# Lcressot/fhe-string-bounty

Hardware: AMD Instinct MI355X
Metric: PBS/sec (whole node) (higher is better)
Workload: dtype f64

## Files before the change

### fhe-string-bounty_amd/csrc/engine.h

```cpp
#pragma once
#include <hip/hip_runtime.h>
#include <stdint.h>

#include <map>
#include <mutex>
#include <string>
#include <vector>

#include "../../include/fhestr.h"

#define FHESTR_KERNEL_REVISION "r04.2"

namespace fhe {

inline uint32_t n_ggsw(const fhe_params_t& p) {
    return p.grouping_factor > 1 ? p.n / p.grouping_factor * (1u << p.grouping_factor) : p.n;
}
inline uint64_t multi_bit_key_bit(const uint64_t* group_bits, uint32_t g, uint32_t sel) {
    uint64_t prod = 1;
    for (uint32_t b = 0; b < g; b++) prod *= group_bits[b] ^ (((sel >> (g - 1 - b)) & 1) ^ 1);
    return prod;
}

void aes128_round_keys(const uint8_t key[16], uint8_t rk[11][16]);
const uint8_t* aes_sbox();

extern thread_local std::string g_last_error;
int fail(const std::string& msg);

struct BrVariant;

uint64_t fill_accumulator(const fhe_params_t& p, const uint64_t* table, std::vector<uint64_t>& acc);
void fill_accumulator_torus(const fhe_params_t& p, const uint64_t* box_values, std::vector<uint64_t>& acc);

struct EngineEnv {
    int log2_points = 0;
    int wide_fair = -1;
    int keep_busy = -1;
    int overlap_streams = -1;
    int ks_mfma = -1;
    int ks_chunks = -1;
    int cluster_mode = -2;
    int cluster_spin_limit = -1;
    int multibit_combine_max = -1;
    int cluster_test_fault = -1;
    int dense_per_cu = -1;
    int cluster_fallback = -1;
    static EngineEnv read();
};

struct Engine {
    std::recursive_mutex mu;
    fhe_params_t p{};
    int device = 0;
    hipStream_t stream = nullptr;
    hipStream_t own_stream = nullptr;
    std::map<std::vector<uint64_t>, uint32_t> lut_dedup;
    hipEvent_t ev[3] = {nullptr, nullptr, nullptr};
    std::vector<hipEvent_t> ring;
    size_t ring_used = 0;
    const BrVariant* variant = nullptr;
    const BrVariant* variant_large = nullptr;
    int cu_count = 256;
    int pipeline = 0;
    hipStream_t ks_stream = nullptr;
    hipEvent_t pipe_ev[5] = {nullptr, nullptr, nullptr, nullptr, nullptr};
    hipEvent_t pipe_input_ready = nullptr;
    const void* pipe_out[2] = {nullptr, nullptr};
    size_t pipe_out_bytes[2] = {0, 0};
    static constexpr int OVL_MAX = 4;
    int ovl_streams = 2;
    uint32_t wide_fair_shift = 13;
    uint32_t dense_per_cu = 2;
    bool keep_busy = false;
    hipStream_t ovl_stream[OVL_MAX] = {nullptr, nullptr, nullptr, nullptr};
    hipEvent_t ovl_done[OVL_MAX] = {nullptr, nullptr, nullptr, nullptr};
    struct ByteRange { const char* lo; const char* hi; };
    std::vector<ByteRange> ovl_ins[OVL_MAX], ovl_outs[OVL_MAX];
    uint64_t* ovl_small[OVL_MAX] = {nullptr, nullptr, nullptr, nullptr};
    size_t ovl_cap_small[OVL_MAX] = {0, 0, 0, 0};
    int8_t* ovl_digits[OVL_MAX] = {nullptr, nullptr, nullptr, nullptr};
    size_t ovl_cap_digits[OVL_MAX] = {0, 0, 0, 0};
    int sync_all_streams();
    void end_pipeline_run();
    uint64_t pipe_calls = 0;
    int shadow_fit = -1;
    uint32_t multibit_combine_max = 64;

    uint32_t* d_ksk_packed = nullptr;
    uint64_t* d_ksk_rowsum = nullptr;
    int8_t* d_ksk_mfma = nullptr;
    int8_t* d_ks_digits = nullptr;
    size_t cap_ks_digits = 0;
    bool ks_mfma_enabled = true;
    double* d_fbsk = nullptr;
    double* d_fbsk_dense = nullptr;
    uint64_t* d_luts = nullptr;
    size_t luts_cap = 0;
    uint32_t n_luts = 0;

    uint64_t *d_in = nullptr, *d_small = nullptr, *d_small2 = nullptr, *d_out = nullptr, *d_pool = nullptr;
    uint32_t* d_idx = nullptr;
    uint32_t* d_slot_exp = nullptr;
    size_t multibit_workspace_cap = 0;
    void* d_meta = nullptr;
    void* d_ws = nullptr;
    size_t cap_ws = 0;
    void* d_cluster_ws = nullptr;
    size_t cap_cluster_ws = 0;
    void* d_cluster_ctl = nullptr;
    bool cluster_unchecked = false;
    uint32_t cluster_last = 0;
    bool cluster_fallback = true;
    uint32_t cluster_fallbacks = 0;
    uint32_t cluster_last_error = 0;
    int cluster_mode = -1;
    uint32_t cluster_max_batch = 0xFFFFFFFFu;
    uint32_t ks_chunks_override = 0;
    int xcd_per_cu = -1;
    uint32_t xcd_auto_max = 16;
    uint32_t cluster_spin_limit = 1u << 22;
    uint32_t cluster_test_fault = 0;
    int cluster_check();
    size_t cap_in = 0, cap_small = 0, cap_small2 = 0, cap_out = 0, cap_idx = 0, cap_pool = 0, cap_meta = 0;

    static int create(const fhe_params_t& p, int device, Engine** out);
    ~Engine();
    int use();
    int set_variant(int logR);
    int load_keys(const uint64_t* bsk_std, const uint64_t* ksk);
    int load_seeded_keys(const uint8_t ksk_seed[16], const uint64_t* ksk_bodies, const uint8_t bsk_seed[16], const uint64_t* bsk_bodies,
                         uint64_t* bsk_std_out, uint64_t* ksk_out);
    int expand_seeded_lwe(const uint8_t* seeds, const uint64_t* bodies, uint32_t count, uint64_t* d_out, uint64_t* host_out);
    int generate_keys(const uint64_t* glwe_sk, const uint64_t* small_sk, const uint8_t seed[32],
                      uint64_t* bsk_std_out, uint64_t* ksk_out);
    int install_keys(uint64_t* d_ksk_std, uint64_t* d_bsk_std);
    int convert_polys(const uint64_t* d_std, double* d_out, uint32_t n_polys);
    int cluster_settle(const uint64_t* d_sm, const uint32_t* d_lut_idx, uint64_t* d_big, uint32_t count);
    int probe_slot_exponents();
    uint64_t fill_accumulator(const uint64_t* table, std::vector<uint64_t>& acc) const { return fhe::fill_accumulator(p, table, acc); }
    int lut_upload_dedup(const std::vector<uint64_t>& acc, uint32_t* id);
    int set_stream(hipStream_t s, bool use_own);
    int lut_upload(const uint64_t* acc, uint32_t* id);
    int lut_download(uint32_t id, uint64_t* acc);
    int ensure_batch(uint32_t count);
    int check_lut_idx(const uint32_t* lut_idx, uint32_t count) const;

    int launch_keyswitch(const uint64_t* d_big, uint64_t* d_sm, uint32_t count, hipStream_t on = nullptr, bool shadow = false, int digits_slot = 0);
    int launch_blind_rotate(const uint64_t* d_sm, const uint32_t* d_lut_idx, uint64_t* d_big, uint32_t count, hipStream_t on = nullptr, bool two_per_cu = false);
    bool shadow_keyswitch_fits();
    int ks_pbs_dev(const uint64_t* d_big_in, const uint32_t* d_lut_idx, uint64_t* d_big_out, uint32_t count, bool allow_pipeline = false);
    int ks_pbs_host(const uint64_t* in, const uint32_t* lut_idx, uint64_t* out, uint32_t count);
    int keyswitch_host(const uint64_t* in, uint64_t* out_small, uint32_t count);
    int pbs_host(const uint64_t* in_small, const uint32_t* lut_idx, uint64_t* out, uint32_t count);
    int pbs_ks_host(const uint64_t* in_small, const uint32_t* lut_idx, uint64_t* out_small, uint32_t count);
    int lincomb_dev(const uint64_t* d_pool, const uint32_t* d_off, const uint32_t* d_src,
                    const int32_t* d_coeff, const uint64_t* d_cst, uint64_t* d_out, uint32_t jobs);
    int lincomb_batch_dev(const uint64_t* d_pool, const uint32_t* d_off, const uint32_t* d_src, const int32_t* d_coeff,
                          const uint64_t* d_cst, uint64_t* d_out, uint32_t jobs, uint32_t instances, uint32_t src_slot, uint32_t src_inst,
                          uint32_t out_job, uint32_t out_inst, const uint32_t* d_lut_in, uint32_t* d_lut_out);
    int restride_dev(const uint64_t* d_in, uint64_t* d_out, uint32_t slots, uint32_t instances, uint32_t in_slot, uint32_t in_inst,
                     uint32_t out_slot, uint32_t out_inst);
    int lincomb_host(const uint64_t* pool, uint32_t pool_count, const uint32_t* off, const uint32_t* src,
                     const int32_t* coeff, const uint64_t* cst, uint64_t* out, uint32_t jobs);
    int last_kernel_ms(float ms[2]);
    int kernel_times(double total_ms[2], uint32_t* calls, bool reset);
    int synchronize();
};

int params_supported(const fhe_params_t& p);

}

struct fhe_plan;
struct fhe_engine {
    fhe::Engine* impl;
    std::vector<std::pair<std::string, fhe_plan*>> str_plans;
};
```

### fhe-string-bounty_amd/csrc/pbs_kernels.hip.h

```cpp
#pragma once
#include <type_traits>
#include "negacyclic_fft.hip.h"

namespace fhe {

#ifdef FHESTR_WALL
__device__ unsigned long long g_wall[4096 * 2];
#endif
#ifdef FHESTR_STAMPS
constexpr int STAMP_SEGS = 10;
__device__ unsigned long long g_stamps[4096 * 8 * STAMP_SEGS];
#define FHE_STAMP_DECL unsigned long long stamp_acc[STAMP_SEGS] = {}; unsigned long long stamp_prev = 0
#define FHE_STAMP(idx)                                                                                   \
    do {                                                                                                 \
        __builtin_amdgcn_sched_barrier(0);                                                               \
        unsigned long long _t;                                                                           \
        asm volatile("s_memtime %0\n\ts_waitcnt lgkmcnt(0)" : "=s"(_t)::"memory");                       \
        __builtin_amdgcn_sched_barrier(0);                                                               \
        if ((idx) >= 0) stamp_acc[(idx) < 0 ? 0 : (idx)] += _t - stamp_prev;                             \
        stamp_prev = _t;                                                                                 \
    } while (0)
#else
#define FHE_STAMP_DECL do {} while (0)
#define FHE_STAMP(idx) do {} while (0)
#endif

__device__ uint32_t g_cu_tickets[2048];

struct BlindRotateArgs {
    const uint64_t* lwe_small;
    const uint32_t* lut_idx;
    const uint64_t* luts;
    const double* fbsk;
    uint64_t* lwe_out;
    uint32_t n;
    uint32_t base_log;
    uint32_t batch;
    uint32_t grouping;
    uint32_t fair_shift;
};

__device__ __forceinline__ uint32_t decomp_init_state(uint64_t x, uint32_t bL) {
    uint32_t t = (uint32_t)(x >> (63 - bL));
    return ((t + 1u) >> 1) & ((1u << bL) - 1u);
}
__device__ __forceinline__ int32_t decomp_next_digit(uint32_t& state, uint32_t base_log) {
    const uint32_t mask = (1u << base_log) - 1u;
    uint32_t res = state & mask;
    state >>= base_log;
    uint32_t carry = ((res - 1u) | state) & res;
    carry >>= base_log - 1;
    state += carry;
    return (int32_t)(res - (carry << base_log));
}
__device__ __forceinline__ uint64_t decomp_init_state64(uint64_t x, uint32_t bL) {
    const uint64_t t = x >> (63 - bL);
    return ((t + 1ull) >> 1) & ((1ull << bL) - 1ull);
}
__device__ __forceinline__ int32_t decomp_next_digit64(uint64_t& state, uint32_t base_log) {
    const uint64_t mask = (1ull << base_log) - 1ull;
    uint64_t res = state & mask;
    state >>= base_log;
    uint64_t carry = ((res - 1ull) | state) & res;
    carry >>= base_log - 1;
    state += carry;
    return (int32_t)(uint32_t)(res - (carry << base_log));
}
__device__ __forceinline__ int32_t decomp_single_digit(uint64_t x, uint32_t b) {
    const uint32_t t = (uint32_t)(x >> 32) >> (31 - b);
    const uint32_t res = __builtin_amdgcn_ubfe(t + 1u, 1u, b);
    const uint32_t half = 1u << (b - 1);
    return (int32_t)(res - ((res + (half - 1u)) & (half << 1)));
}
__device__ __forceinline__ uint32_t decomp_bias_constant(uint32_t b) {
    uint32_t c = 0x80000000u - (1u << (31 - b));
    asm volatile("" : "+s"(c));
    return c;
}
__device__ __forceinline__ uint32_t decomp_single_biased(uint64_t x, uint32_t b, uint32_t bias_constant) {
    const uint32_t hi = (uint32_t)(x >> 32);
    return __builtin_amdgcn_ubfe(hi + bias_constant, 32u - b, b);
}
__device__ __forceinline__ cplx digit_point(uint32_t lo_biased, uint32_t hi_biased, cplx tw, cplx kb) {
    const double a = (double)lo_biased, b = (double)hi_biased;
    cplx r;
    r.re = fma(a, tw.re, fma(-b, tw.im, kb.re));
    r.im = fma(a, tw.im, fma(b, tw.re, kb.im));
    return r;
}
__device__ __forceinline__ uint32_t modulus_switch(uint64_t x, int logN) {
    uint64_t o = x >> (64 - logN - 2);
    return (uint32_t)((o + 1) >> 1);
}

typedef unsigned int u32x4_t __attribute__((ext_vector_type(4)));
__device__ __forceinline__ auto key_resource(const double* fbsk, size_t bytes) {
    return __builtin_amdgcn_make_buffer_rsrc(const_cast<double*>(fbsk), 0, bytes < 0x7FFFFFF0u ? (int)bytes : 0x7FFFFFF0, 0x00020000);
}
template <class RSRC>
__device__ __forceinline__ double2 key_load(RSRC rsrc, uint32_t voff, uint32_t soff) {
    const u32x4_t v = __builtin_amdgcn_raw_buffer_load_b128(rsrc, (int)voff, (int)soff, 0);
    double2 d;
    __builtin_memcpy(&d, &v, 16);
    return d;
}

template <class PL>
__device__ __forceinline__ uint32_t acc_slot_of(uint32_t j) { return (uint32_t)PL::acc_slot((int)j); }

template <class PL>
__host__ __device__ constexpr int swap_wave_bits() {
    if constexpr (PL::SWAP) return PL::LOGW; else return 0;
}
template <class PL, int LOGN>
struct Rotation {
    int32_t oddmask;
    uint32_t rem;
    int32_t qb8;
    uint32_t rbits8;
    __device__ __forceinline__ Rotation(uint32_t d, int tau) {
        rem = d & ((1u << LOGN) - 1);
        oddmask = -(int32_t)((d >> LOGN) & 1);
        if constexpr (PL::SWAP) {
            constexpr int LW = swap_wave_bits<PL>();
            const int w = __builtin_amdgcn_readfirstlane(tau >> 6), lane = tau & 63;
            const int rr = (int)(rem & ((1u << LW) - 1));
            qb8 = (int32_t)((uint32_t)((lane - (int)(rem >> LW) - (w < rr ? 1 : 0)) << 3) + ((uint32_t)oddmask & 0x80000000u));
            rbits8 = (uint32_t)((w - rr) & ((1 << LW) - 1)) << (LOGN - LW + 3);
        } else {
            qb8 = 0; rbits8 = 0;
        }
    }
    __device__ __forceinline__ void source(int tau, int m, int h, uint32_t& slot, uint32_t& neg) const {
        static_assert(!PL::SWAP, "swap plan: use source_bytes");
        const uint32_t j = (uint32_t)PL::point(tau, m) + (uint32_t)h * PL::P;
        neg = (uint32_t)(((int32_t)(j - rem) >> 31) ^ oddmask);
        slot = acc_slot_of<PL>((j - rem) & ((1u << LOGN) - 1));
    }
    __device__ __forceinline__ void source_bytes(int m, int h, uint32_t row_base, uint32_t& address, uint32_t& neg) const {
        constexpr int LW = swap_wave_bits<PL>();
        const int32_t q8 = qb8 + ((PL::point(0, m) + h * PL::P) >> LW) * 8;
        neg = (uint32_t)(q8 >> 31);
        address = ((uint32_t)q8 & (((1u << (LOGN - LW)) - 1) << 3)) | row_base;
    }
    __device__ __forceinline__ void source_bytes_q8(int m, int h, uint32_t row_base, uint32_t& address, int32_t& q8) const {
        constexpr int LW = swap_wave_bits<PL>();
        q8 = qb8 + ((PL::point(0, m) + h * PL::P) >> LW) * 8;
        address = ((uint32_t)q8 & (((1u << (LOGN - LW)) - 1) << 3)) | row_base;
    }
};

__device__ __forceinline__ uint32_t biased_difference(uint64_t gathered, int32_t q8, uint64_t own_nk, uint32_t b) {
    const uint32_t sm = (uint32_t)(q8 >> 31), nsm = ~sm;
    const uint64_t s = gathered + (own_nk ^ (((uint64_t)nsm << 32) | nsm));
    return __builtin_amdgcn_ubfe((uint32_t)(s >> 32) ^ sm, 32u - b, b);
}

typedef __attribute__((address_space(3))) const uint64_t lds_cu64_t;
__device__ __forceinline__ uint32_t lds_address(const void* p) {
    return (uint32_t)(uintptr_t)(__attribute__((address_space(3))) const void*)p;
}
__device__ __forceinline__ uint64_t lds_load_u64(uint32_t byte_address) { return *(lds_cu64_t*)(uintptr_t)byte_address; }

template <int LOGN, int LOGR, int K1, int L>
struct BrCfg {
    static constexpr int N = 1 << LOGN;
    static constexpr int P = N / 2;
    using PL = typename PlanFor<LOGN - 1, LOGR>::type;
    static constexpr int R = PL::R;
    static constexpr int T = PL::T;
    static constexpr int THREADS = K1 * T;
    static constexpr int PLANE = P + 2;
    static constexpr int GROUP_SLOTS = 2 * P + 4;
    static constexpr size_t LDS_FIXED = (size_t)K1 * N * 8  + (size_t)K1 * GROUP_SLOTS * 8  +
                                        (size_t)K1 * GROUP_SLOTS * 8 ;
    static size_t lds_bytes(uint32_t n) { return LDS_FIXED + (size_t)n * 4; }
};

template <int LOGN, int LOGR, int K1, int L>
__global__ void __launch_bounds__((BrCfg<LOGN, LOGR, K1, L>::THREADS))
bsk_convert_kernel(const uint64_t* __restrict__ bsk_std, double* __restrict__ fbsk, uint32_t n_polys) {
    using CFG = BrCfg<LOGN, LOGR, K1, L>;
    using PL = typename CFG::PL;
    constexpr int N = CFG::N, P = CFG::P, R = CFG::R, T = CFG::T;
    extern __shared__ __align__(16) unsigned char smem[];
    const int g = threadIdx.x / T, tau = threadIdx.x % T;
    double* xre = reinterpret_cast<double*>(smem) + (size_t)g * CFG::GROUP_SLOTS;
    double* xim = xre + CFG::PLANE;
    const uint32_t poly = blockIdx.x * K1 + g;
    const bool active = poly < n_polys;
    FftConsts<PL> fc;
    fft_init_consts<PL>(fc, tau);
    cplx x[R];
#pragma unroll
    for (int m = 0; m < R; m++) {
        const int j = PL::point(tau, m);
        uint64_t a = active ? bsk_std[(size_t)poly * N + j] : 0;
        uint64_t b = active ? bsk_std[(size_t)poly * N + j + P] : 0;
        cplx z;
        z.re = i64_to_f64(a) * (5.421010862427522e-20 / P);
        z.im = i64_to_f64(b) * (5.421010862427522e-20 / P);
        double sn, cs;
        sincospi((double)j / (double)N, &sn, &cs);
        cplx w; w.re = cs; w.im = sn;
        x[m] = cmul(z, w);
    }
    fft_forward<PL>(x, fc, xre, xim, tau);
    if (active) {
        double2* out = reinterpret_cast<double2*>(fbsk) + (size_t)poly * P;
#pragma unroll
        for (int rho = 0; rho < R; rho++) out[rho * T + tau] = make_double2(x[rho].re, x[rho].im);
    }
}

template <int LOGN, int LOGR, int K1, int L, bool EXTPROD = false>
__global__ void __launch_bounds__((BrCfg<LOGN, LOGR, K1, L>::THREADS))
blind_rotate_kernel(BlindRotateArgs args) {
    using CFG = BrCfg<LOGN, LOGR, K1, L>;
    static_assert(!EXTPROD || !CFG::PL::SWAP, "N = 2048 has its own multi-bit kernels");
    using PL = typename CFG::PL;
    constexpr int N = CFG::N, P = CFG::P, R = CFG::R, T = CFG::T;
    extern __shared__ __align__(16) unsigned char smem[];
    uint64_t* lds_acc = reinterpret_cast<uint64_t*>(smem);
    double* lds_x = reinterpret_cast<double*>(smem + (size_t)K1 * N * 8);
    double* lds_f = lds_x + (size_t)K1 * CFG::GROUP_SLOTS;
    uint32_t* lds_d = reinterpret_cast<uint32_t*>(lds_f + (size_t)K1 * CFG::GROUP_SLOTS);

    int g = threadIdx.x / T;
    const int tau = threadIdx.x % T;
    if constexpr (T % 64 == 0) g = __builtin_amdgcn_readfirstlane(g);
#ifdef FHESTR_WALL
    const unsigned long long wall_t0 = __builtin_amdgcn_s_memrealtime();
#endif
    const uint32_t sample = blockIdx.x < args.batch ? blockIdx.x : blockIdx.x % args.batch;
    const uint32_t n = args.n;
    const uint64_t* lwe = args.lwe_small + (size_t)sample * (n + 1);
    const uint64_t* lut = args.luts + (size_t)(args.lut_idx ? args.lut_idx[sample] : 0) * K1 * N;
    uint64_t* my_acc = lds_acc + (size_t)g * N;
    const uint32_t my_acc_address = lds_address(my_acc);
    if (PL::SWAP && (my_acc_address & (8u * N - 1u))) __builtin_trap();
    double* xre = lds_x + (size_t)g * CFG::GROUP_SLOTS;
    double* xim = xre + CFG::PLANE;
    const uint32_t bL = args.base_log * L;
    const uint32_t dbias = decomp_bias_constant(bL <= 31 ? bL : 31);

    const uint32_t steps = EXTPROD ? n / args.grouping : n;
    for (uint32_t i = threadIdx.x; i < steps; i += CFG::THREADS) {
        const uint64_t a = lwe[i];
        lds_d[i] = EXTPROD ? 0u : (a == 0 ? 0xFFFFFFFFu : modulus_switch(a, LOGN));
    }

    FftConsts<PL> fc;
    fft_init_consts<PL>(fc, tau);
    cplx twist[R], twbias[R];
#pragma unroll
    for (int m = 0; m < R; m++) {
        double sn, cs;
        sincospi((double)PL::point(tau, m) / (double)N, &sn, &cs);
        twist[m].re = cs; twist[m].im = sn;
        const double cb = -(double)((1u << (args.base_log * L - 1)) - 1u);
        twbias[m].re = cb * (cs - sn);
        twbias[m].im = cb * (cs + sn);
    }

    uint64_t acc_lo[R], acc_hi[R];
    {
        const uint32_t d = modulus_switch(lwe[n], LOGN);
        const uint32_t rem = d & (N - 1);
        const bool odd = (d >> LOGN) & 1;
#pragma unroll
        for (int m = 0; m < R; m++) {
#pragma unroll
            for (int h = 0; h < 2; h++) {
                const uint32_t j = PL::point(tau, m) + h * P;
                const uint32_t src = (j + rem) & (N - 1);
                const bool neg = ((j + rem) >= (uint32_t)N) != odd;
                uint64_t v = lut[(size_t)g * N + src];
                v = neg ? (0 - v) : v;
                if (h == 0) acc_lo[m] = v; else acc_hi[m] = v;
            }
        }
    }
#pragma unroll
    for (int m = 0; m < R; m++) {
        my_acc[acc_slot_of<PL>(PL::point(tau, m))] = acc_lo[m];
        my_acc[acc_slot_of<PL>(PL::point(tau, m) + P)] = acc_hi[m];
    }
    __syncthreads();

    const double2* fbsk = reinterpret_cast<const double2*>(args.fbsk);
    constexpr size_t GGSW_ELEMS = (size_t)L * K1 * K1 * P;

    uint32_t d_next = lds_d[0];
    const uint32_t key_off = (uint32_t)tau * 16u;
    if constexpr (EXTPROD) fbsk += (size_t)sample * steps * GGSW_ELEMS;
    const auto key_rsrc = key_resource(reinterpret_cast<const double*>(fbsk), (size_t)steps * GGSW_ELEMS * 16);
    FHE_STAMP_DECL;
    FHE_STAMP(-1);
    for (uint32_t i = 0; i < steps; i++) {
        const uint32_t d = (uint32_t)__builtin_amdgcn_readfirstlane((int)d_next);
        d_next = lds_d[i + 1 < steps ? i + 1 : i];
        if (d == 0xFFFFFFFFu) continue;
        const Rotation<PL, LOGN> rot(d, tau);

        const double2* bk0 = fbsk + (size_t)i * GGSW_ELEMS;
        double2 bpre[K1][R];
        {
#pragma unroll
            for (int r = 0; r < K1; r++) {
                const int row = (g + r) % K1;
#pragma unroll
                for (int rho = 0; rho < R; rho++) {
                    const uint32_t soff = (uint32_t)((i * GGSW_ELEMS + (size_t)(L - 1) * K1 * K1 * P +
                                                      ((size_t)row * K1 + g) * P + rho * T) * 16);
                    bpre[r][rho] = key_load(key_rsrc, key_off, soff);
                }
            }
        }

        uint32_t st_lo[R], st_hi[R];
        uint32_t row_base = my_acc_address | rot.rbits8;
        if constexpr (PL::SWAP) asm volatile("" : "+s"(row_base));
#pragma unroll
        for (int m = 0; m < R; m++) {
#pragma unroll
            for (int h = 0; h < 2; h++) {
                if constexpr (EXTPROD) {
                    const uint64_t own = h == 0 ? acc_lo[m] : acc_hi[m];
                    const uint32_t st = L == 1 ? decomp_single_biased(own, bL, dbias) : decomp_init_state(own, bL);
                    if (h == 0) st_lo[m] = st; else st_hi[m] = st;
                    continue;
                }
                uint32_t sm32;
                uint64_t gathered;
                if constexpr (PL::SWAP) {
                    uint32_t address;
                    rot.source_bytes(m, h, row_base, address, sm32);
                    gathered = lds_load_u64(address);
                } else {
                    uint32_t slot;
                    rot.source(tau, m, h, slot, sm32);
                    gathered = my_acc[slot];
                }
                const uint64_t sm = ((uint64_t)sm32 << 32) | sm32;
                const uint64_t v = (gathered ^ sm) - sm;
                const uint64_t own = h == 0 ? acc_lo[m] : acc_hi[m];
                const uint32_t st = L == 1 ? decomp_single_biased(v - own, bL, dbias) : decomp_init_state(v - own, bL);
                if (h == 0) st_lo[m] = st; else st_hi[m] = st;
            }
        }

        FHE_STAMP(0);
        cplx outf[R];
        if constexpr (PL::SWAP) {
            static_assert(!PL::SWAP || L == 1, "swap plan: single decomposition level only");
            cplx x[K1][R];
#pragma unroll
            for (int m = 0; m < R; m++) x[0][m] = digit_point(st_lo[m], st_hi[m], twist[m], twbias[m]);
#ifdef FHESTR_WALL
    if (threadIdx.x == 0 && blockIdx.x < 4096) {
        uint32_t xcc;
        asm volatile("s_getreg_b32 %0, hwreg(HW_REG_XCC_ID)" : "=s"(xcc));
        g_wall[blockIdx.x * 2] = __builtin_amdgcn_s_memrealtime() - wall_t0;
        g_wall[blockIdx.x * 2 + 1] = xcc & 7u;
    }
#endif
#ifdef FHESTR_STAMPS
            swap10_fwd_stage1(x[0], fc, xre, xim, tau);
            FHE_STAMP(1);
            wave_local_fence();
            swap10_fwd_stage2(x[0], fc, xre, xim, tau);
            FHE_STAMP(2);
            wave_local_fence();
            swap10_fwd_stage3(x[0], fc, xre, xim, tau);
            FHE_STAMP(3);
#else
            swap10_forward_head(x[0], fc, xre, xim, tau);
#endif
            __syncthreads();
            FHE_STAMP(4);
#pragma unroll
            for (int r = 0; r < K1; r++) {
                const int row = (g + r) % K1;
                const double* rre = lds_x + (size_t)row * CFG::GROUP_SLOTS;
                swap10_forward_tail(x[r], rre, rre + CFG::PLANE, tau);
            }
#pragma unroll
            for (int r = 0; r < K1; r++) {
#pragma unroll
                for (int rho = 0; rho < R; rho++) {
                    const double2 bv = bpre[r][rho];
                    const cplx f = x[r][rho];
                    if (r == 0) {
                        outf[rho].re = bv.x * f.re - bv.y * f.im;
                        outf[rho].im = bv.x * f.im + bv.y * f.re;
                    } else {
                        outf[rho].re = fma(bv.x, f.re, fma(-bv.y, f.im, outf[rho].re));
                        outf[rho].im = fma(bv.x, f.im, fma(bv.y, f.re, outf[rho].im));
                    }
                }
            }
            double* fre = lds_f + (size_t)g * CFG::GROUP_SLOTS;
            double* fim = fre + CFG::PLANE;
            FHE_STAMP(5);
            swap10_inverse_head(outf, fre, fim, tau);
            FHE_STAMP(6);
            __syncthreads();
            FHE_STAMP(7);
            swap10_inverse_tail(outf, fc, fre, fim, tau);
            FHE_STAMP(8);
        } else {
#pragma unroll
        for (int it = 0; it < L; it++) {
            const int lvl_idx = L - 1 - it;
            cplx x[R];
#pragma unroll
            for (int m = 0; m < R; m++) {
                if (L == 1) { x[m] = digit_point(st_lo[m], st_hi[m], twist[m], twbias[m]); continue; }
                cplx z;
                z.re = (double)decomp_next_digit(st_lo[m], args.base_log);
                z.im = (double)decomp_next_digit(st_hi[m], args.base_log);
                x[m] = cmul(z, twist[m]);
            }
            fft_forward<PL>(x, fc, xre, xim, tau);
            if (it > 0) __syncthreads();
            {
                double* fre = lds_f + (size_t)g * CFG::GROUP_SLOTS;
                double* fim = fre + CFG::PLANE;
#pragma unroll
                for (int rho = 0; rho < R; rho++) {
                    fre[rho * T + tau] = x[rho].re;
                    fim[rho * T + tau] = x[rho].im;
                }
            }
            __syncthreads();
            const double2* bk = bk0 + (size_t)lvl_idx * K1 * K1 * P;
#pragma unroll
            for (int r = 0; r < K1; r++) {
                const int row = (g + r) % K1;
                const double* fre = lds_f + (size_t)row * CFG::GROUP_SLOTS;
                const double* fim = fre + CFG::PLANE;
#pragma unroll
                for (int rho = 0; rho < R; rho++) {
                    const double2 bv = it == 0 ? bpre[r][rho] : bk[((size_t)row * K1 + g) * P + rho * T + tau];
                    cplx f;
                    if (r == 0) {
                        f = x[rho];
                    } else {
                        f.re = fre[rho * T + tau];
                        f.im = fim[rho * T + tau];
                    }
                    if (it == 0 && r == 0) {
                        outf[rho].re = bv.x * f.re - bv.y * f.im;
                        outf[rho].im = bv.x * f.im + bv.y * f.re;
                    } else {
                        outf[rho].re = fma(bv.x, f.re, fma(-bv.y, f.im, outf[rho].re));
                        outf[rho].im = fma(bv.x, f.im, fma(bv.y, f.re, outf[rho].im));
                    }
                }
            }
        }

        fft_inverse<PL>(outf, fc, xre, xim, tau);
        }
#pragma unroll
        for (int m = 0; m < R; m++) {
            cplx t = cmul_conj(outf[m], twist[m]);
            if constexpr (EXTPROD) {
                acc_lo[m] = from_torus(t.re);
                acc_hi[m] = from_torus(t.im);
                continue;
            }
            acc_lo[m] += from_torus(t.re);
            acc_hi[m] += from_torus(t.im);
            my_acc[acc_slot_of<PL>(PL::point(tau, m))] = acc_lo[m];
            my_acc[acc_slot_of<PL>(PL::point(tau, m) + P)] = acc_hi[m];
            FHE_PIN_ORDER();
        }
        __syncthreads();
        FHE_STAMP(9);
    }
#ifdef FHESTR_STAMPS
    if ((threadIdx.x & 63) == 0 && blockIdx.x < 4096)
        for (int sg = 0; sg < STAMP_SEGS; sg++)
            g_stamps[((size_t)blockIdx.x * 8 + (threadIdx.x >> 6)) * STAMP_SEGS + sg] = stamp_acc[sg];
#endif

    if (blockIdx.x >= args.batch) return;
    uint64_t* out = args.lwe_out + (size_t)sample * ((size_t)(K1 - 1) * N + 1);
#pragma unroll
    for (int m = 0; m < R; m++) {
#pragma unroll
        for (int h = 0; h < 2; h++) {
            const uint32_t j = PL::point(tau, m) + h * P;
            const uint64_t v = h == 0 ? acc_lo[m] : acc_hi[m];
            if (g == K1 - 1) {
                if (j == 0) out[(size_t)(K1 - 1) * N] = v;
            } else {
                if (j == 0) out[(size_t)g * N] = v;
                else out[(size_t)g * N + (N - j)] = 0 - v;
            }
        }
    }
}

#ifndef FHESTR_SWAP11
#define FHESTR_SWAP11 1
#endif
#ifndef FHESTR_WIDE_SWAP9
#define FHESTR_WIDE_SWAP9 0
#endif
template <int LOGN, int LOGR, int K1, int L, bool KEYPF = false>
struct BrWideCfg {
    static constexpr int N = 1 << LOGN;
    static constexpr int P = N / 2;
    static constexpr bool OWN_PLAN = (FHESTR_SWAP11 && LOGN == 12 && LOGR == 2) || (FHESTR_WIDE_SWAP9 && LOGN == 10 && LOGR == 2);
    static constexpr bool LDS_TWIDDLES = OWN_PLAN && LOGN == 12;
    using PL = typename std::conditional<!OWN_PLAN, typename PlanFor<LOGN - 1, LOGR>::type,
                                         typename std::conditional<LOGN == 12, FftSwap11, FftSwap9>::type>::type;
    static constexpr int R = PL::R;
    static constexpr int T = PL::T;
    static constexpr int THREADS = T;
    static constexpr int PLANE = P + 2;
    static constexpr int GROUP_SLOTS = 2 * P + 4;
    static constexpr bool TW_IN_LDS = !PL::SWAP && PL::NTW > 4;
    static constexpr size_t LDS_TW = TW_IN_LDS ? (size_t)FftHybridConsts<PL>::ENTRIES * 16
                                     : LDS_TWIDDLES ? (size_t)FftSwapLdsConsts<PL>::ENTRIES * 16 : 0;
    static constexpr size_t LDS_FIXED = (size_t)K1 * N * 8  + (size_t)K1 * GROUP_SLOTS * 8  + LDS_TW;
#ifndef FHESTR_WIDE_ACC_LDS_LOGN
#define FHESTR_WIDE_ACC_LDS_LOGN 12
#endif
    static constexpr bool ACC_IN_LDS = LOGN >= FHESTR_WIDE_ACC_LDS_LOGN;
    static constexpr bool PREFETCH_ALL = K1 * K1 * R * 4 <= 64 || KEYPF;
    static constexpr bool ROW_BATCH = !PREFETCH_ALL && OWN_PLAN && L == 1;
};

template <int LOGN, int LOGR, int K1, int L, bool KEYPF = false>
__global__ void __launch_bounds__((BrWideCfg<LOGN, LOGR, K1, L, KEYPF>::THREADS))
blind_rotate_wide_kernel(BlindRotateArgs args) {
    using CFG = BrWideCfg<LOGN, LOGR, K1, L, KEYPF>;
    using PL = typename CFG::PL;
    constexpr int N = CFG::N, P = CFG::P, R = CFG::R, T = CFG::T;
    extern __shared__ __align__(16) unsigned char smem[];
    uint64_t* lds_acc = reinterpret_cast<uint64_t*>(smem);
    double* lds_x = reinterpret_cast<double*>(smem + (size_t)K1 * N * 8);
    double2* lds_tw = reinterpret_cast<double2*>(lds_x + (size_t)K1 * CFG::GROUP_SLOTS);
    uint32_t* lds_d = reinterpret_cast<uint32_t*>(lds_tw + CFG::LDS_TW / 16);

    const int tau = threadIdx.x;
#ifdef FHESTR_WALL
    const unsigned long long wall_t0 = __builtin_amdgcn_s_memrealtime();
#endif
    const uint32_t sample = blockIdx.x;
    const uint32_t n = args.n;
    const uint64_t* lwe = args.lwe_small + (size_t)sample * (n + 1);
    const uint64_t* lut = args.luts + (size_t)(args.lut_idx ? args.lut_idx[sample] : 0) * K1 * N;
    const uint32_t acc_address = lds_address(lds_acc);
    if (PL::SWAP && (acc_address & (8u * N - 1u))) __builtin_trap();
    const uint32_t bL = args.base_log * L;
    const uint32_t dbias = decomp_bias_constant(bL <= 31 ? bL : 31);
    if (args.fair_shift && threadIdx.x == 0) {
        uint32_t fair_parity;
        uint32_t hw, xcc;
        asm volatile("s_getreg_b32 %0, hwreg(HW_REG_HW_ID)" : "=s"(hw));
        asm volatile("s_getreg_b32 %0, hwreg(HW_REG_XCC_ID)" : "=s"(xcc));
        fair_parity = atomicAdd(&g_cu_tickets[((xcc & 7u) << 8) | ((hw >> 8) & 0xFFu)], 1u) & 1u;
        reinterpret_cast<uint32_t*>(lds_x)[0] = fair_parity;
    }

    for (uint32_t i = threadIdx.x; i < n; i += CFG::THREADS) {
        const uint64_t a = lwe[i];
        lds_d[i] = a == 0 ? 0xFFFFFFFFu : modulus_switch(a, LOGN);
    }

    typename std::conditional<CFG::LDS_TWIDDLES, FftSwapLdsConsts<PL>,
                              typename std::conditional<CFG::TW_IN_LDS, FftHybridConsts<PL>, FftConsts<PL>>::type>::type fc;
    if constexpr (CFG::LDS_TWIDDLES) {
        FftSwapLdsConsts<PL>::fill(lds_tw, threadIdx.x, CFG::THREADS);
        fc.init(lds_tw, tau);
    } else if constexpr (CFG::TW_IN_LDS) {
        FftHybridConsts<PL>::fill(lds_tw, threadIdx.x, CFG::THREADS);
        fc.init(lds_tw, tau);
    } else {
        fft_init_consts<PL>(fc, tau);
    }
    cplx twist[R], twbias[R];
#pragma unroll
    for (int m = 0; m < R; m++) {
        double sn, cs;
        sincospi((double)PL::point(tau, m) / (double)N, &sn, &cs);
        twist[m].re = cs; twist[m].im = sn;
        const double cb = -(double)((1u << (args.base_log * L - 1)) - 1u);
        twbias[m].re = cb * (cs - sn);
        twbias[m].im = cb * (cs + sn);
    }

    constexpr bool ACC_LDS = CFG::ACC_IN_LDS;
    uint64_t acc_lo[ACC_LDS ? 1 : K1][R], acc_hi[ACC_LDS ? 1 : K1][R];
    auto own_slot = [&](int p, int m, int h) { return (size_t)p * N + acc_slot_of<PL>(PL::point(tau, m) + h * P); };
    {
        const uint32_t d = modulus_switch(lwe[n], LOGN);
        const uint32_t rem = d & (N - 1);
        const bool odd = (d >> LOGN) & 1;
#pragma unroll
        for (int p = 0; p < K1; p++)
#pragma unroll
            for (int m = 0; m < R; m++)
#pragma unroll
                for (int h = 0; h < 2; h++) {
                    const uint32_t j = PL::point(tau, m) + h * P;
                    const uint32_t src = (j + rem) & (N - 1);
                    const bool neg = ((j + rem) >= (uint32_t)N) != odd;
                    uint64_t v = lut[(size_t)p * N + src];
                    v = neg ? (0 - v) : v;
                    if constexpr (!ACC_LDS) { if (h == 0) acc_lo[p][m] = v; else acc_hi[p][m] = v; }
                    lds_acc[(size_t)p * N + acc_slot_of<PL>(j)] = v;
                }
    }
    __syncthreads();

    const double2* fbsk = reinterpret_cast<const double2*>(args.fbsk);
    constexpr size_t GGSW_ELEMS = (size_t)L * K1 * K1 * P;
    const uint32_t key_off = (uint32_t)tau * 16u;
    const auto key_rsrc = key_resource(args.fbsk, (size_t)n * GGSW_ELEMS * 16);

    const uint32_t fair_shift = args.fair_shift;
    uint32_t fair_turn = 0;
    if (fair_shift) {
        fair_turn = (uint32_t)__builtin_amdgcn_readfirstlane((int)reinterpret_cast<uint32_t*>(lds_x)[0]);
        __syncthreads();
    }
    uint32_t d_next = lds_d[0];
    for (uint32_t i = 0; i < n; i++) {
        const uint32_t d = (uint32_t)__builtin_amdgcn_readfirstlane((int)d_next);
        d_next = lds_d[i + 1 < n ? i + 1 : i];
        if (d == 0xFFFFFFFFu) continue;
        if (fair_shift) {
            if ((((uint32_t)(__builtin_amdgcn_s_memrealtime() >> fair_shift)) ^ fair_turn) & 1u) __builtin_amdgcn_s_setprio(1);
            else __builtin_amdgcn_s_setprio(0);
        }
        const Rotation<PL, LOGN> rot(d, tau);
        const double2* bk0 = fbsk + (size_t)i * GGSW_ELEMS;

        double2 bpre[CFG::PREFETCH_ALL ? K1 : 1][CFG::PREFETCH_ALL ? K1 : 1][R];
        if (CFG::PREFETCH_ALL) {
#pragma unroll
            for (int row = 0; row < K1; row++)
#pragma unroll
                for (int col = 0; col < K1; col++)
#pragma unroll
                    for (int rho = 0; rho < R; rho++)
                        bpre[row][col][rho] = key_load(key_rsrc, key_off,
                            (uint32_t)((i * GGSW_ELEMS + (size_t)(L - 1) * K1 * K1 * P + ((size_t)row * K1 + col) * P + rho * T) * 16));
        }

        uint32_t st_lo[K1][R], st_hi[K1][R];
        const uint64_t nk = ~((uint64_t)dbias << 32);
        uint32_t row_base[K1];
#pragma unroll
        for (int p = 0; p < K1; p++) {
            row_base[p] = (acc_address + (uint32_t)p * 8u * N) | rot.rbits8;
            if constexpr (PL::SWAP) asm volatile("" : "+s"(row_base[p]));
        }
        constexpr bool GATHER_BATCH = PL::SWAP && L == 1 && !ACC_LDS;
        if constexpr (GATHER_BATCH) {
            uint64_t gv[K1][R][2];
            int32_t q8v[R][2];
#pragma unroll
            for (int m = 0; m < R; m++)
#pragma unroll
                for (int h = 0; h < 2; h++) {
                    uint32_t address;
                    rot.source_bytes_q8(m, h, row_base[0], address, q8v[m][h]);
#pragma unroll
                    for (int p = 0; p < K1; p++) gv[p][m][h] = lds_load_u64(address + (uint32_t)p * 8u * N);
                }
            FHE_PIN_ORDER();
#pragma unroll
            for (int p = 0; p < K1; p++)
#pragma unroll
                for (int m = 0; m < R; m++) {
                    st_lo[p][m] = biased_difference(gv[p][m][0], q8v[m][0], acc_lo[p][m] + nk, bL);
                    st_hi[p][m] = biased_difference(gv[p][m][1], q8v[m][1], acc_hi[p][m] + nk, bL);
                }
        }
#pragma unroll
        for (int p = 0; p < (GATHER_BATCH ? 0 : K1); p++)
#pragma unroll
            for (int m = 0; m < R; m++)
#pragma unroll
                for (int h = 0; h < 2; h++) {
                    uint32_t sm32;
                    uint64_t gathered;
                    if constexpr (PL::SWAP) {
                        uint32_t address;
                        rot.source_bytes(m, h, row_base[p], address, sm32);
                        gathered = lds_load_u64(address);
                    } else {
                        uint32_t slot;
                        rot.source(tau, m, h, slot, sm32);
                        gathered = lds_acc[(size_t)p * N + slot];
                    }
                    const uint64_t sm = ((uint64_t)sm32 << 32) | sm32;
                    const uint64_t v = (gathered ^ sm) - sm;
                    uint64_t own;
                    if constexpr (ACC_LDS) own = lds_acc[own_slot(p, m, h)];
                    else own = h == 0 ? acc_lo[p][m] : acc_hi[p][m];
                    const uint32_t st = L == 1 ? decomp_single_biased(v - own, bL, dbias) : decomp_init_state(v - own, bL);
                    if (h == 0) st_lo[p][m] = st; else st_hi[p][m] = st;
                }

        cplx outf[K1][R];
#pragma unroll
        for (int it = 0; it < L; it++) {
            const int lvl_idx = L - 1 - it;
            cplx x[K1][R];
#pragma unroll
            for (int p = 0; p < K1; p++)
#pragma unroll
                for (int m = 0; m < R; m++) {
                    if (L == 1) {
                        if constexpr (CFG::LDS_TWIDDLES) {
                            const int32_t cbi = (int32_t)((1u << (args.base_log * L - 1)) - 1u);
                            cplx z;
                            z.re = (double)((int32_t)st_lo[p][m] - cbi);
                            z.im = (double)((int32_t)st_hi[p][m] - cbi);
                            x[p][m] = cmul(z, twist[m]);
                        } else {
                            x[p][m] = digit_point(st_lo[p][m], st_hi[p][m], twist[m], twbias[m]);
                        }
                        continue;
                    }
                    cplx z;
                    z.re = (double)decomp_next_digit(st_lo[p][m], args.base_log);
                    z.im = (double)decomp_next_digit(st_hi[p][m], args.base_log);
                    x[p][m] = cmul(z, twist[m]);
                }
            fft_forward_multi<PL, K1>(x, fc, lds_x, CFG::GROUP_SLOTS, CFG::PLANE, tau);
            const double2* bk = bk0 + (size_t)lvl_idx * K1 * K1 * P;
#pragma unroll
            for (int row = 0; row < K1; row++) {
                double2 krow[CFG::ROW_BATCH ? K1 : 1][CFG::ROW_BATCH ? R : 1];
                if constexpr (CFG::ROW_BATCH) {
#pragma unroll
                    for (int col = 0; col < K1; col++)
#pragma unroll
                        for (int rho = 0; rho < R; rho++)
                            krow[col][rho] = key_load(key_rsrc, key_off,
                                (uint32_t)((i * GGSW_ELEMS + (size_t)lvl_idx * K1 * K1 * P + ((size_t)row * K1 + col) * P + rho * T) * 16));
                    FHE_PIN_ORDER();
                }
#pragma unroll
                for (int col = 0; col < K1; col++)
#pragma unroll
                    for (int rho = 0; rho < R; rho++) {
                        const double2 bv = CFG::ROW_BATCH ? krow[CFG::ROW_BATCH ? col : 0][CFG::ROW_BATCH ? rho : 0]
                                           : (CFG::PREFETCH_ALL && it == 0)
                                               ? bpre[CFG::PREFETCH_ALL ? row : 0][CFG::PREFETCH_ALL ? col : 0][rho]
                                               : bk[((size_t)row * K1 + col) * P + rho * T + tau];
                        const cplx f = x[row][rho];
                        if (it == 0 && row == 0) {
                            outf[col][rho].re = bv.x * f.re - bv.y * f.im;
                            outf[col][rho].im = bv.x * f.im + bv.y * f.re;
                        } else {
                            outf[col][rho].re = fma(bv.x, f.re, fma(-bv.y, f.im, outf[col][rho].re));
                            outf[col][rho].im = fma(bv.x, f.im, fma(bv.y, f.re, outf[col][rho].im));
                        }
                    }
            }
            if (it + 1 < L) __syncthreads();
        }

        fft_inverse_multi<PL, K1>(outf, fc, lds_x, CFG::GROUP_SLOTS, CFG::PLANE, tau);
#pragma unroll
        for (int p = 0; p < K1; p++)
#pragma unroll
            for (int m = 0; m < R; m++) {
                cplx t = cmul_conj(outf[p][m], twist[m]);
                if constexpr (ACC_LDS) {
                    lds_acc[own_slot(p, m, 0)] += from_torus(t.re);
                    lds_acc[own_slot(p, m, 1)] += from_torus(t.im);
                } else {
                acc_lo[p][m] += from_torus(t.re);
                acc_hi[p][m] += from_torus(t.im);
                lds_acc[(size_t)p * N + acc_slot_of<PL>(PL::point(tau, m))] = acc_lo[p][m];
                lds_acc[(size_t)p * N + acc_slot_of<PL>(PL::point(tau, m) + P)] = acc_hi[p][m];
                }
                FHE_PIN_ORDER();
            }
        __syncthreads();
    }

#ifdef FHESTR_WALL
    if (threadIdx.x == 0 && blockIdx.x < 4096) {
        g_wall[blockIdx.x * 2] = __builtin_amdgcn_s_memrealtime() - wall_t0;
        g_wall[blockIdx.x * 2 + 1] = wall_t0;
    }
#endif
    uint64_t* out = args.lwe_out + (size_t)sample * ((size_t)(K1 - 1) * N + 1);
#pragma unroll
    for (int p = 0; p < K1; p++)
#pragma unroll
        for (int m = 0; m < R; m++)
#pragma unroll
            for (int h = 0; h < 2; h++) {
                const uint32_t j = PL::point(tau, m) + h * P;
                uint64_t v;
                if constexpr (ACC_LDS) v = lds_acc[own_slot(p, m, h)];
                else v = h == 0 ? acc_lo[p][m] : acc_hi[p][m];
                if (p == K1 - 1) {
                    if (j == 0) out[(size_t)(K1 - 1) * N] = v;
                } else {
                    if (j == 0) out[(size_t)p * N] = v;
                    else out[(size_t)p * N + (N - j)] = 0 - v;
                }
            }
}

template <int LOGN, int LOGR, int K1, int L>
__global__ void __launch_bounds__((BrWideCfg<LOGN, LOGR, K1, L>::THREADS))
bsk_convert_wide_kernel(const uint64_t* __restrict__ bsk_std, double* __restrict__ fbsk, uint32_t n_polys) {
    using CFG = BrWideCfg<LOGN, LOGR, K1, L>;
    using PL = typename CFG::PL;
    constexpr int N = CFG::N, P = CFG::P, R = CFG::R, T = CFG::T;
    extern __shared__ __align__(16) unsigned char smem[];
    double* planes = reinterpret_cast<double*>(smem);
    const int tau = threadIdx.x;
    const uint32_t poly = blockIdx.x;
    if (poly >= n_polys) return;
    FftConsts<PL> fc;
    fft_init_consts<PL>(fc, tau);
    cplx x[R];
#pragma unroll
    for (int m = 0; m < R; m++) {
        const int j = PL::point(tau, m);
        const uint64_t a = bsk_std[(size_t)poly * N + j];
        const uint64_t b = bsk_std[(size_t)poly * N + j + P];
        cplx z;
        z.re = i64_to_f64(a) * (5.421010862427522e-20 / P);
        z.im = i64_to_f64(b) * (5.421010862427522e-20 / P);
        double sn, cs;
        sincospi((double)j / (double)N, &sn, &cs);
        cplx w; w.re = cs; w.im = sn;
        x[m] = cmul(z, w);
    }
    fft_forward<PL>(x, fc, planes, planes + CFG::PLANE, tau);
    double2* out = reinterpret_cast<double2*>(fbsk) + (size_t)poly * P;
#pragma unroll
    for (int rho = 0; rho < R; rho++) out[rho * T + tau] = make_double2(x[rho].re, x[rho].im);
}

}
```

Measured before the change: 131,600.

## Add overlapped wide blind-rotate loop with early key loads and split FFT stages

Adds a specialized blind-rotate loop for the swap10 FFT plan with K1=2, L=1 and prefetched keys. It issues all bootstrapping-key loads at the top of each iteration so they overlap the decomposition and forward FFT, and interleaves the per-row DFT and key multiply with the inverse FFT head. It also sets waves_per_eu to 2 for this config. Timestamp instrumentation is extended and compiled out by default. The cost is more registers for the held key rows, which could spill under the two-wave occupancy target.

Result: faster. 133,700 (median of 6 runs) (+1.5%).

```diff
diff --git a/fhe-string-bounty_amd/csrc/engine.h b/fhe-string-bounty_amd/csrc/engine.h
--- a/fhe-string-bounty_amd/csrc/engine.h
+++ b/fhe-string-bounty_amd/csrc/engine.h
@@ -9,7 +9,7 @@
 
 #include "../../include/fhestr.h"
 
-#define FHESTR_KERNEL_REVISION "r04.2"
+#define FHESTR_KERNEL_REVISION "r04.3"
 
 namespace fhe {
 
diff --git a/fhe-string-bounty_amd/csrc/pbs_kernels.hip.h b/fhe-string-bounty_amd/csrc/pbs_kernels.hip.h
--- a/fhe-string-bounty_amd/csrc/pbs_kernels.hip.h
+++ b/fhe-string-bounty_amd/csrc/pbs_kernels.hip.h
@@ -8,7 +8,7 @@
 __device__ unsigned long long g_wall[4096 * 2];
 #endif
 #ifdef FHESTR_STAMPS
-constexpr int STAMP_SEGS = 10;
+constexpr int STAMP_SEGS = 16;
 __device__ unsigned long long g_stamps[4096 * 8 * STAMP_SEGS];
 #define FHE_STAMP_DECL unsigned long long stamp_acc[STAMP_SEGS] = {}; unsigned long long stamp_prev = 0
 #define FHE_STAMP(idx)                                                                                   \
@@ -20,9 +20,11 @@
         if ((idx) >= 0) stamp_acc[(idx) < 0 ? 0 : (idx)] += _t - stamp_prev;                             \
         stamp_prev = _t;                                                                                 \
     } while (0)
+#define FHE_STAMP_VMWAIT() asm volatile("s_waitcnt vmcnt(0)" ::: "memory")
 #else
 #define FHE_STAMP_DECL do {} while (0)
 #define FHE_STAMP(idx) do {} while (0)
+#define FHE_STAMP_VMWAIT() do {} while (0)
 #endif
 
 __device__ uint32_t g_cu_tickets[2048];
@@ -509,6 +511,9 @@
 #endif
 #ifndef FHESTR_WIDE_SWAP9
 #define FHESTR_WIDE_SWAP9 0
+#endif
+#ifndef FHESTR_WIDE_OVERLAP
+#define FHESTR_WIDE_OVERLAP 1
 #endif
 template <int LOGN, int LOGR, int K1, int L, bool KEYPF = false>
 struct BrWideCfg {
@@ -533,10 +538,13 @@
     static constexpr bool ACC_IN_LDS = LOGN >= FHESTR_WIDE_ACC_LDS_LOGN;
     static constexpr bool PREFETCH_ALL = K1 * K1 * R * 4 <= 64 || KEYPF;
     static constexpr bool ROW_BATCH = !PREFETCH_ALL && OWN_PLAN && L == 1;
+    static constexpr bool OVERLAP = FHESTR_WIDE_OVERLAP && std::is_same<PL, FftSwap10>::value && K1 == 2 && L == 1 && PREFETCH_ALL &&
+                                    !ACC_IN_LDS;
 };
 
 template <int LOGN, int LOGR, int K1, int L, bool KEYPF = false>
 __global__ void __launch_bounds__((BrWideCfg<LOGN, LOGR, K1, L, KEYPF>::THREADS))
+__attribute__((amdgpu_waves_per_eu(BrWideCfg<LOGN, LOGR, K1, L, KEYPF>::OVERLAP ? 2 : 1)))
 blind_rotate_wide_kernel(BlindRotateArgs args) {
     using CFG = BrWideCfg<LOGN, LOGR, K1, L, KEYPF>;
     using PL = typename CFG::PL;
@@ -631,7 +639,142 @@
         __syncthreads();
     }
     uint32_t d_next = lds_d[0];
-    for (uint32_t i = 0; i < n; i++) {
+    FHE_STAMP_DECL;
+    FHE_STAMP(-1);
+    constexpr bool OVERLAP = CFG::OVERLAP;
+    if constexpr (OVERLAP) {
+        double2 bk[K1][K1][R];
+        auto load_row = [&](uint32_t s, int row) {
+#pragma unroll
+            for (int col = 0; col < K1; col++)
+#pragma unroll
+                for (int rho = 0; rho < R; rho++)
+                    bk[row][col][rho] = key_load(key_rsrc, key_off, (uint32_t)((s * GGSW_ELEMS + ((size_t)row * K1 + col) * P + rho * T) * 16));
+        };
+        auto re_of = [&](int p) { return lds_x + (size_t)p * CFG::GROUP_SLOTS; };
+        auto im_of = [&](int p) { return lds_x + (size_t)p * CFG::GROUP_SLOTS + CFG::PLANE; };
+        for (uint32_t i = 0; i < n; i++) {
+            const uint32_t d = (uint32_t)__builtin_amdgcn_readfirstlane((int)d_next);
+            d_next = lds_d[i + 1 < n ? i + 1 : i];
+            if (d == 0xFFFFFFFFu) continue;
+            if (fair_shift) {
+                if ((((uint32_t)(__builtin_amdgcn_s_memrealtime() >> fair_shift)) ^ fair_turn) & 1u) __builtin_amdgcn_s_setprio(1);
+                else __builtin_amdgcn_s_setprio(0);
+            }
+            FHE_STAMP(11);
+            load_row(i, 0);
+            load_row(i, 1);
+            const Rotation<PL, LOGN> rot(d, tau);
+            uint32_t row_base = acc_address | rot.rbits8;
+            asm volatile("" : "+s"(row_base));
+            uint64_t gv[K1][R][2];
+            int32_t q8v[R][2];
+#pragma unroll
+            for (int m = 0; m < R; m++)
+#pragma unroll
+                for (int h = 0; h < 2; h++) {
+                    uint32_t address;
+                    rot.source_bytes_q8(m, h, row_base, address, q8v[m][h]);
+#pragma unroll
+                    for (int p = 0; p < K1; p++) gv[p][m][h] = lds_load_u64(address + (uint32_t)p * 8u * N);
+                }
+            FHE_PIN_ORDER();
+            const uint64_t nk = ~((uint64_t)dbias << 32);
+            cplx x[K1][R];
+#pragma unroll
+            for (int p = 0; p < K1; p++)
+#pragma unroll
+                for (int m = 0; m < R; m++) {
+                    const uint32_t st_lo = biased_difference(gv[p][m][0], q8v[m][0], acc_lo[p][m] + nk, bL);
+                    const uint32_t st_hi = biased_difference(gv[p][m][1], q8v[m][1], acc_hi[p][m] + nk, bL);
+                    x[p][m] = digit_point(st_lo, st_hi, twist[m], twbias[m]);
+                }
+            FHE_STAMP(0);
+#pragma unroll
+            for (int p = 0; p < K1; p++) swap10_fwd_stage1(x[p], fc, re_of(p), im_of(p), tau);
+            wave_local_fence();
+#pragma unroll
+            for (int p = 0; p < K1; p++) swap10_fwd_stage2(x[p], fc, re_of(p), im_of(p), tau);
+            wave_local_fence();
+#pragma unroll
+            for (int p = 0; p < K1; p++) swap10_fwd_stage3(x[p], fc, re_of(p), im_of(p), tau);
+            FHE_STAMP(1);
+            __syncthreads();
+            FHE_STAMP(2);
+#pragma unroll
+            for (int p = 0; p < K1; p++)
+#pragma unroll
+                for (int r = 0; r < 4; r++) {
+                    const int a = swap10_comb(tau, r);
+                    x[p][r].re = re_of(p)[a];
+                    x[p][r].im = im_of(p)[a];
+                }
+            FHE_PIN_ORDER();
+            FHE_STAMP(3);
+            FHE_STAMP_VMWAIT();
+            FHE_STAMP(4);
+            cplx outf[K1][R];
+            small_dft<4, false>(x[0]);
+#pragma unroll
+            for (int col = 0; col < K1; col++)
+#pragma unroll
+                for (int rho = 0; rho < R; rho++) {
+                    const double2 bv = bk[0][col][rho];
+                    const cplx f = x[0][rho];
+                    outf[col][rho].re = bv.x * f.re - bv.y * f.im;
+                    outf[col][rho].im = bv.x * f.im + bv.y * f.re;
+                }
+            small_dft<4, false>(x[1]);
+#pragma unroll
+            for (int col = 0; col < K1; col++) {
+#pragma unroll
+                for (int rho = 0; rho < R; rho++) {
+                    const double2 bv = bk[1][col][rho];
+                    const cplx f = x[1][rho];
+                    outf[col][rho].re = fma(bv.x, f.re, fma(-bv.y, f.im, outf[col][rho].re));
+                    outf[col][rho].im = fma(bv.x, f.im, fma(bv.y, f.re, outf[col][rho].im));
+                }
+                swap10_inverse_head(outf[col], re_of(col), im_of(col), tau);
+            }
+            FHE_STAMP(5);
+            __syncthreads();
+            FHE_STAMP(6);
+#pragma unroll
+            for (int p = 0; p < K1; p++)
+#pragma unroll
+                for (int r = 0; r < 4; r++) {
+                    const int a = swap10_slab(tau, r);
+                    outf[p][r].re = re_of(p)[a];
+                    outf[p][r].im = im_of(p)[a];
+                }
+            FHE_PIN_ORDER();
+            FHE_STAMP(7);
+#pragma unroll
+            for (int p = 0; p < K1; p++) swap10_inv_stage1_compute(outf[p], fc);
+            wave_local_fence();
+#pragma unroll
+            for (int p = 0; p < K1; p++) swap10_inv_stage2(outf[p], fc, re_of(p), im_of(p), tau);
+            wave_local_fence();
+#pragma unroll
+            for (int p = 0; p < K1; p++) swap10_inv_stage3(outf[p], fc, re_of(p), im_of(p), tau);
+            FHE_STAMP(8);
+#pragma unroll
+            for (int p = 0; p < K1; p++)
+#pragma unroll
+                for (int m = 0; m < R; m++) {
+                    cplx t = cmul_conj(outf[p][m], twist[m]);
+                    acc_lo[p][m] += from_torus(t.re);
+                    acc_hi[p][m] += from_torus(t.im);
+                    lds_acc[(size_t)p * N + acc_slot_of<PL>(PL::point(tau, m))] = acc_lo[p][m];
+                    lds_acc[(size_t)p * N + acc_slot_of<PL>(PL::point(tau, m) + P)] = acc_hi[p][m];
+                    FHE_PIN_ORDER();
+                }
+            FHE_STAMP(9);
+            __syncthreads();
+            FHE_STAMP(10);
+        }
+    }
+    for (uint32_t i = 0; i < (OVERLAP ? 0u : n); i++) {
         const uint32_t d = (uint32_t)__builtin_amdgcn_readfirstlane((int)d_next);
         d_next = lds_d[i + 1 < n ? i + 1 : i];
         if (d == 0xFFFFFFFFu) continue;
@@ -639,6 +782,7 @@
             if ((((uint32_t)(__builtin_amdgcn_s_memrealtime() >> fair_shift)) ^ fair_turn) & 1u) __builtin_amdgcn_s_setprio(1);
             else __builtin_amdgcn_s_setprio(0);
         }
+        FHE_STAMP(11);
         const Rotation<PL, LOGN> rot(d, tau);
         const double2* bk0 = fbsk + (size_t)i * GGSW_ELEMS;
 
@@ -709,6 +853,7 @@
                     const uint32_t st = L == 1 ? decomp_single_biased(v - own, bL, dbias) : decomp_init_state(v - own, bL);
                     if (h == 0) st_lo[p][m] = st; else st_hi[p][m] = st;
                 }
+        FHE_STAMP(0);
 
         cplx outf[K1][R];
 #pragma unroll
@@ -737,6 +882,9 @@
                     x[p][m] = cmul(z, twist[m]);
                 }
             fft_forward_multi<PL, K1>(x, fc, lds_x, CFG::GROUP_SLOTS, CFG::PLANE, tau);
+            FHE_STAMP(1);
+            FHE_STAMP_VMWAIT();
+            FHE_STAMP(4);
             const double2* bk = bk0 + (size_t)lvl_idx * K1 * K1 * P;
 #pragma unroll
             for (int row = 0; row < K1; row++) {
@@ -770,8 +918,10 @@
             }
             if (it + 1 < L) __syncthreads();
         }
+        FHE_STAMP(5);
 
         fft_inverse_multi<PL, K1>(outf, fc, lds_x, CFG::GROUP_SLOTS, CFG::PLANE, tau);
+        FHE_STAMP(8);
 #pragma unroll
         for (int p = 0; p < K1; p++)
 #pragma unroll
@@ -788,8 +938,15 @@
                 }
                 FHE_PIN_ORDER();
             }
+        FHE_STAMP(9);
         __syncthreads();
-    }
+        FHE_STAMP(10);
+    }
+#ifdef FHESTR_STAMPS
+    if ((threadIdx.x & 63) == 0 && blockIdx.x < 4096)
+        for (int sg = 0; sg < STAMP_SEGS; sg++)
+            g_stamps[((size_t)blockIdx.x * 8 + (threadIdx.x >> 6)) * STAMP_SEGS + sg] = stamp_acc[sg];
+#endif
 
 #ifdef FHESTR_WALL
     if (threadIdx.x == 0 && blockIdx.x < 4096) {
```
